# upb-lea/gym-electric-motor

Hardware: AMD Instinct MI355X
Metric: env-steps/sec (batched PMSM, tau=1e-4) (higher is better)
Workload: dtype f32; 1 GPU; Finite-CC-PMSM-v0 (Finite-B6C + dq transform), RK4, fp32, tau=1e-4, default constraint + auto-reset; 16384 envs/GPU x 1 GPU(s); one bench step = one fused launch of 1000 control steps, obs [K,N,S_out] rows + done bytes written for every control step; env_id=Finite-CC-PMSM-v0, envs_per_gpu=16384, solver=rk4, steps_per_launch=1000, parallelism=env-sharded x1, no data-path collective, world_size=1, oversubscribed=False

## Files before the change

### gym_electric_motor_amd/csrc/gemx_kernels.hpp

```cpp
#pragma once
#include <cstdio>

#include "gemx_common.hpp"

namespace gemx {

__device__ __forceinline__ float med3_r(float x, float lo, float hi) { return __builtin_amdgcn_fmed3f(x, lo, hi); }
__device__ __forceinline__ double med3_r(double x, double lo, double hi) { return fmin(fmax(x, lo), hi); }
template <class R> __device__ __forceinline__ R poly_load_ode(const DevParams<R> &P, R omega, R torque) {
    const R a = med3_r(P.lin_factor * omega, -P.la, P.la);
    const R tl = P.lc * (omega * fabs(omega)) + P.lb * omega + a;
    return (torque - tl) * P.inv_j;
}

template <int SYS, class R> struct Elec;

template <class R> struct Elec<GEMX_SYS_DC_PERMEX, R> {
    static constexpr int NM = 1;
    struct Pre { R b; };
    static __device__ __forceinline__ Pre prep(const DevParams<R> &P, R w, const R (&u)[MAX_U]) {
        const R bw = P.m[0] * w;
        return Pre{fma(P.m[2], u[0], bw)};
    }
    static __device__ __forceinline__ void f(const DevParams<R> &P, const Pre &p, const R (&x)[1], R (&dx)[1]) { dx[0] = p.b + P.m[1] * x[0]; }
// ... 485 lines not shown
                rhs(z, k1);
                wsum += rk_step_k1_pk<SOLVER, NP>(z, k1, hs, rhs);
            }
        }
        put();
        return P.pole * hs * wsum;
    }
    float deps = 0.0f;
    const float lim = P.omega_lim;
    const float h_td = hs * P.inv_tau_decay;
    for (int s = 0; s < (NS1 ? 1 : ns); ++s) {
        V k1;
        rhs(z, k1);
        const float w = z.w;
        const float wmid = fmaf(0.5f * hs, k1.w, w);
        const bool band = fabsf(wmid) < lim;
        const float c1 = band ? P.lin_factor : 0.0f, c0 = band ? 0.0f : copysignf(P.la, wmid);
        k1.w = fmaf(med3_r(P.lin_factor * w, -P.la, P.la) - fmaf(c1, w, c0), P.inv_j, k1.w);
        auto rhs_m = [&](const V &zz, V &dz) {
            const float om = zz.w;
            dz.w = (E.rhs(P, zz, dz) - (P.lc * (om * fabsf(om)) + P.lb * om + fmaf(c1, om, c0))) * P.inv_j;
        };
        float dw_end;
        deps += (P.pole * hs) * rk_step_k1_pk<SOLVER, NP>(z, k1, hs, rhs_m, &dw_end);
        const float w1 = z.w;
        const float phi_lim = copysignf(lim, wmid);
        const bool needs = (med3_r(w, -lim, lim) != (band ? w : phi_lim)) | (med3_r(w1, -lim, lim) != (band ? w1 : phi_lim));
        if (__any(needs)) {
            const float V0 = hs * k1.w, V1 = hs * dw_end, dl = w1 - w;
            const float c2 = 3.0f * dl - 2.0f * V0 - V1, c3 = V0 + V1 - 2.0f * dl;
            const KinkPath<float> kp{w, w1, V0, V0 * V0, 4.0f * (dl - V0), c2 * (1.0f / 3.0f), c3 * 0.25f, 0.5f * V0,
                                     w + 0.5f * V0 + c2 * (1.0f / 3.0f) + c3 * 0.25f, w1 > w};
            const float lev = (kp.up ? (w < -lim) : !(w > lim)) ? -lim : lim, oth = -lev;
            const float U1 = kp.ramp(lev);
            const bool o0 = w >= oth, o1 = w1 >= oth, full = o0 != o1;
            float U2 = (o0 & o1) ? kp.M - oth : 0.0f;
            if (__any(full)) {
                const float uf = kp.ramp(oth);
                U2 = full ? uf : U2;
            }
            const float Up = lev > 0.0f ? U1 : U2, Um = lev > 0.0f ? U2 : U1;
            const float D = -h_td * ((Um - Up - lim) - (band ? kp.M : phi_lim));
            z.w = w1 + (needs ? D : 0.0f);
        }
    }
    put();
    return deps;
}

template <int SYS>
__device__ __forceinline__ float dp5_adaptive_pk(const DevParams<float> &P, float (&y)[SysTraits<SYS>::ND], const float (&u)[MAX_U], float hs, float *hc) {
    constexpr int NP = pk_pairs<SYS>(), NZ = 1 + 2 * NP;
    using V = PkVec<NP>;
    const PkElec<SYS> E(P, u);
    V z, k1;
    z.w = y[0];
#pragma unroll
    for (int j = 0; j < NP; ++j) z.p[j] = f2_t{y[1 + 2 * j], y[2 + 2 * j]};
    auto rhs = [&](const V &zz, V &dz) { dz.w = poly_load_ode<float>(P, zz.w, E.rhs(P, zz, dz)); };
    const bool kink = P.kink_split != 0;
    V k1t;
    rhs(z, k1t);
    float t = 0.0f, h = dp5_first_try<float>(P, hs, hc), integral = 0.0f, hprop = 0.0f;
    const float hmin = hs * (1.0f / 1024.0f);
    bool gave_up = false;
#pragma nounroll
    for (int guard = 0; guard < 4096; ++guard) {
        const bool active = t < hs;
        if (!__any(active)) break;
        const bool fin = !(h < hs - t);
        const float hh = active ? (fin ? hs - t : h) : 0.0f;
        V k2, k3, k4, k5, k6, k7, zt, zn;
        k1 = k1t;
        float kc0 = 0.0f, kc1 = 0.0f, wmid = 0.0f;
        bool band = false;
        if (kink) {
            wmid = fmaf(0.5f * hh, k1t.w, z.w);
            band = fabsf(wmid) < P.omega_lim;
            kc1 = band ? P.lin_factor : 0.0f;
            kc0 = band ? 0.0f : copysignf(P.la, wmid);
            k1.w = fmaf(med3_r(P.lin_factor * z.w, -P.la, P.la) - fmaf(kc1, z.w, kc0), P.inv_j, k1t.w);
        }
        auto ev = [&](const V &zz, V &dz) {
            const float tq = E.rhs(P, zz, dz);
            const float om = zz.w;
            if (kink) dz.w = (tq - (P.lc * (om * fabsf(om)) + P.lb * om + fmaf(kc1, om, kc0))) * P.inv_j;
            else dz.w = poly_load_ode<float>(P, om, tq);
        };
        float q = (float)(35.0 / 384.0) * z.w;
        zt = pk_axpy(z, hh, pk_scale((float)(1.0 / 5.0), k1));
        ev(zt, k2);
        zt = pk_axpy(z, hh, pk_acc(pk_scale((float)(3.0 / 40.0), k1), (float)(9.0 / 40.0), k2));
        ev(zt, k3);
        q += (float)(500.0 / 1113.0) * zt.w;
        zt = pk_axpy(z, hh, pk_acc(pk_acc(pk_scale((float)(44.0 / 45.0), k1), -(float)(56.0 / 15.0), k2), (float)(32.0 / 9.0), k3));
        ev(zt, k4);
        q += (float)(125.0 / 192.0) * zt.w;
        zt = pk_axpy(z, hh, pk_acc(pk_acc(pk_acc(pk_scale((float)(19372.0 / 6561.0), k1), -(float)(25360.0 / 2187.0), k2), (float)(64448.0 / 6561.0), k3),
                                   -(float)(212.0 / 729.0), k4));
        ev(zt, k5);
        q -= (float)(2187.0 / 6784.0) * zt.w;
        zt = pk_axpy(z, hh, pk_acc(pk_acc(pk_acc(pk_acc(pk_scale((float)(9017.0 / 3168.0), k1), -(float)(355.0 / 33.0), k2), (float)(46732.0 / 5247.0), k3),
                                          (float)(49.0 / 176.0), k4), -(float)(5103.0 / 18656.0), k5));
        ev(zt, k6);
        q += (float)(11.0 / 84.0) * zt.w;
        zn = pk_axpy(z, hh, pk_acc(pk_acc(pk_acc(pk_acc(pk_scale((float)(35.0 / 384.0), k1), (float)(500.0 / 1113.0), k3), (float)(125.0 / 192.0), k4),
                                          -(float)(2187.0 / 6784.0), k5), (float)(11.0 / 84.0), k6));
        ev(zn, k7);
        const V er = pk_scale(hh, pk_acc(pk_acc(pk_acc(pk_acc(pk_acc(pk_scale((float)(71.0 / 57600.0), k1), -(float)(71.0 / 16695.0), k3), (float)(71.0 / 1920.0), k4),
                                                        -(float)(17253.0 / 339200.0), k5), (float)(22.0 / 525.0), k6), -(float)(1.0 / 40.0), k7));
        auto sq = [&](float e, float a0, float a1, float at) { const float r = e * rcp_r(at + P.rtol * fmaxf(fabsf(a0), fabsf(a1))); return r * r; };
        float e2 = sq(er.w, z.w, zn.w, P.atol_w);
#pragma unroll
        for (int j = 0; j < NP; ++j) e2 += sq(er.p[j].x, z.p[j].x, zn.p[j].x, P.atol) + sq(er.p[j].y, z.p[j].y, zn.p[j].y, P.atol);
        const float en2 = e2 * (1.0f / NZ);
        const bool floor_hit = !(hh > hmin);
        const bool accept = active && (!(en2 > 1.0f) || floor_hit);
        gave_up |= active && floor_hit && en2 > 1.0f;
        float fac = en2 > 1e-20f ? 0.9f * pow_m01(en2) : 10.0f;
        fac = fminf(fmaxf(fac, 0.2f), accept ? 10.0f : 1.0f);
        const float w0 = z.w;
        z.w = accept ? zn.w : z.w;
        k1t.w = accept ? k7.w : k1t.w;
#pragma unroll
        for (int j = 0; j < NP; ++j) {
            z.p[j] = accept ? zn.p[j] : z.p[j];
            k1t.p[j] = accept ? k7.p[j] : k1t.p[j];
        }
        if (kink) {
            const float lim = P.omega_lim, phi_lim = copysignf(lim, wmid), w1 = zn.w;
            const bool needs = accept && ((med3_r(w0, -lim, lim) != (band ? w0 : phi_lim)) | (med3_r(w1, -lim, lim) != (band ? w1 : phi_lim)));
            if (__any(needs)) {
                z.w = z.w + kink_defect<float>(P, w0, w1, hh * k1.w, hh * k7.w, wmid, band, needs, hh);
                V kt;
                rhs(z, kt);
                k1t.w = needs ? kt.w : k1t.w;
#pragma unroll
                for (int j = 0; j < NP; ++j) k1t.p[j] = needs ? kt.p[j] : k1t.p[j];
            }
        }
        integral += accept ? hh * q : 0.0f;
        t = accept ? (fin ? hs : t + hh) : t;
        h = active ? fmaxf(hh * fac, hmin) : h;
        hprop = accept ? fmaxf(hprop, h) : hprop;
    }
    if (gave_up && P.errw != nullptr) atomicOr(P.errw, (uint32_t)GEMX_ERRFLAG_TOLERANCE);
    if (dp5_carries<float>(P, hs, hc)) *hc = hprop;
    y[0] = z.w;
#pragma unroll
    for (int j = 0; j < NP; ++j) { y[1 + 2 * j] = z.p[j].x; y[2 + 2 * j] = z.p[j].y; }
    return integral;
}

template <int SYS, int LOAD, int SOLVER, class R, bool NS1 = false, bool LIN = false, int SEG = 0>
__device__ __forceinline__ R integrate(const DevParams<R> &P, R (&y)[SysTraits<SYS>::ND], const R (&u)[MAX_U], R h, const R *linr = nullptr, bool two = false,
                                       R *hc = nullptr) {
    using E = Elec<SYS, R>;
    constexpr int NM = E::NM;
    const int ns = NS1 ? 1 : P.nsteps;
    const R hs = NS1 ? h : h * P.inv_ns;
    if (LIN) {
        constexpr int NG = E::NG;
        R g[NG], x[NM];
        constexpr int NC = NM * (NM + NG);
        const R *L0 = linr != nullptr ? linr : P.lin + (SEG != 0 ? NC : 0);
        R L[NC];
        [[maybe_unused]] uint32_t two_mask = (SEG == 1 && two) ? 0xFFFFFFFFu : 0u;
        if constexpr (SEG == 1 && sizeof(R) == 4) asm volatile("" : "+v"(two_mask));
#pragma unroll
        for (int i = 0; i < NC; ++i) {
            if constexpr (SEG == 1 && sizeof(R) == 4) {
                uint32_t ca, cb;
                memcpy(&ca, &L0[2 * NC + i], 4);
                memcpy(&cb, &L0[i], 4);
                const uint32_t cs = (two_mask & cb) | (~two_mask & ca);
                memcpy(&L[i], &cs, 4);
            } else if constexpr (SEG == 1) {
                L[i] = two ? L0[i] : L0[2 * NC + i];
            } else {
                L[i] = L0[SEG == 2 ? NC + i : i];
            }
        }
        const R om = P.init[0];
        E::get_b(E::prep(P, om, u), g);
#pragma unroll
        for (int i = 0; i < NM; ++i) x[i] = y[1 + i];
        for (int s = 0; s < ns; ++s) {
            R xn[NM];
#pragma unroll
            for (int r = 0; r < NM; ++r) {
                constexpr bool X_FIRST = SEG == 0 && (SYS == GEMX_SYS_SYNC || SYS == GEMX_SYS_SCIM);
                constexpr bool X_LAST = !lin_phi_form<SYS, SEG>() && !X_FIRST;
                R acc = X_FIRST ? fma(L[NM * NM + r * NG], g[0], x[r]) : L[NM * NM + r * NG] * g[0];
#pragma unroll
                for (int i = 1; i < NG; ++i) acc += L[NM * NM + r * NG + i] * g[i];
#pragma unroll
                for (int c = 0; c < NM; ++c) acc += L[r * NM + c] * x[c];
                xn[r] = X_LAST ? x[r] + acc : acc;
            }
#pragma unroll
            for (int r = 0; r < NM; ++r) x[r] = xn[r];
        }
#pragma unroll
        for (int i = 0; i < NM; ++i) y[1 + i] = x[i];
        return P.pole * om * h;
    }
    if (LOAD == GEMX_LOAD_CONST_SPEED) {
        const typename E::Pre pre = E::prep(P, y[0], u);
        R x[NM];
#pragma unroll
        for (int i = 0; i < NM; ++i) x[i] = y[1 + i];
        auto rhs = [&](const R (&xx)[NM], R (&dx)[NM]) { E::f(P, pre, xx, dx); };
        if (SOLVER == GEMX_SOLVER_DP5 && P.adaptive) {
            dp5_adaptive<NM, R>(P, x, h, rhs, hc);
        } else if (NS1 || ns == 1) {
            rk_step<SOLVER, NM, R>(x, hs, rhs);
        } else {
            for (int s = 0; s < ns; ++s) rk_step<SOLVER, NM, R>(x, hs, rhs);
        }
#pragma unroll
        for (int i = 0; i < NM; ++i) y[1 + i] = x[i];
        return P.pole * y[0] * h;
    } else {
        if constexpr (sizeof(R) == 4 && pk_pairs<SYS>() > 0 && GEMX_PACKED_RHS) {
            if (!(SOLVER == GEMX_SOLVER_DP5 && P.adaptive)) return integrate_pk<SYS, SOLVER, NS1>(P, y, u, hs, ns);
            if constexpr (SOLVER == GEMX_SOLVER_DP5) return P.pole * dp5_adaptive_pk<SYS>(P, y, u, h, hc);
        }
        auto rhs = [&](const R (&z)[NM + 1], R (&dz)[NM + 1]) {
            R x[NM], dx[NM];
#pragma unroll
            for (int i = 0; i < NM; ++i) x[i] = z[1 + i];
            const typename E::Pre pre = E::prep(P, z[0], u);
            E::f(P, pre, x, dx);
            dz[0] = poly_load_ode(P, z[0], E::torque(P, x));
#pragma unroll
            for (int i = 0; i < NM; ++i) dz[1 + i] = dx[i];
        };
        if (SOLVER == GEMX_SOLVER_DP5 && P.adaptive) {
            auto rhs_mc = [&](const R (&z)[NM + 1], R (&dz)[NM + 1], R c0, R c1) {
                R x[NM], dx[NM];
#pragma unroll
                for (int i = 0; i < NM; ++i) x[i] = z[1 + i];
                const typename E::Pre pre = E::prep(P, z[0], u);
                E::f(P, pre, x, dx);
                dz[0] = (E::torque(P, x) - (P.lc * (z[0] * fabs(z[0])) + P.lb * z[0] + fma(c1, z[0], c0))) * P.inv_j;
#pragma unroll
                for (int i = 0; i < NM; ++i) dz[1 + i] = dx[i];
            };
            return P.pole * dp5_adaptive<NM + 1, R>(P, y, h, rhs, hc, rhs_mc);
        }
        if (!P.kink_split) {
            R wsum = R(0);
            if (NS1 || ns == 1) {
                wsum = rk_step<SOLVER, NM + 1, R>(y, hs, rhs);
            } else {
                for (int s = 0; s < ns; ++s) wsum += rk_step<SOLVER, NM + 1, R>(y, hs, rhs);
            }
            return P.pole * hs * wsum;
        }
        R deps = R(0);
        const R lim = P.omega_lim;
        const R h_td = hs * P.inv_tau_decay;
        for (int s = 0; s < ns; ++s) {
            R k1[NM + 1];
            rhs(y, k1);
            const R w = y[0];
            const R wmid = fma(R(0.5) * hs, k1[0], w);
            const bool band = fabs(wmid) < lim;
            const R c1 = band ? P.lin_factor : R(0), c0 = band ? R(0) : copysign(P.la, wmid);
            k1[0] = fma(med3_r(P.lin_factor * w, -P.la, P.la) - fma(c1, w, c0), P.inv_j, k1[0]);
            auto load_m = [&](R om, R torque) { return (torque - (P.lc * (om * fabs(om)) + P.lb * om + fma(c1, om, c0))) * P.inv_j; };
            auto rhs_m = [&](const R (&z)[NM + 1], R (&dz)[NM + 1]) {
                R x[NM], dx[NM];
#pragma unroll
                for (int i = 0; i < NM; ++i) x[i] = z[1 + i];
                const typename E::Pre pre = E::prep(P, z[0], u);
                E::f(P, pre, x, dx);
                dz[0] = load_m(z[0], E::torque(P, x));
#pragma unroll
                for (int i = 0; i < NM; ++i) dz[1 + i] = dx[i];
            };
            R dw_end;
            deps += (P.pole * hs) * rk_step_k1<SOLVER, NM + 1, R>(y, k1, hs, rhs_m, &dw_end);
            const R w1 = y[0];
            const R phi_lim = copysign(lim, wmid);
            const bool needs = (med3_r(w, -lim, lim) != (band ? w : phi_lim)) | (med3_r(w1, -lim, lim) != (band ? w1 : phi_lim));
#ifdef GEMX_KINK_NO_DEFECT
            if (false) {
#else
            if (__any(needs)) {
#endif
                const R V0 = hs * k1[0], V1 = hs * dw_end, dl = w1 - w;
                const R c2 = R(3) * dl - R(2) * V0 - V1, c3 = V0 + V1 - R(2) * dl;
                const KinkPath<R> kp{w, w1, V0, V0 * V0, R(4) * (dl - V0), c2 * R(1.0 / 3.0), c3 * R(0.25), R(0.5) * V0,
                                     w + R(0.5) * V0 + c2 * R(1.0 / 3.0) + c3 * R(0.25), w1 > w};
                const R lev = (kp.up ? (w < -lim) : !(w > lim)) ? -lim : lim, oth = -lev;
                const R U1 = kp.ramp(lev);
                const bool o0 = w >= oth, o1 = w1 >= oth, full = o0 != o1;
                R U2 = (o0 & o1) ? kp.M - oth : R(0);
                if (__any(full)) {
                    const R uf = kp.ramp(oth);
                    U2 = full ? uf : U2;
                }
                const R Up = lev > R(0) ? U1 : U2, Um = lev > R(0) ? U2 : U1;
                const R D = -h_td * ((Um - Up - lim) - (band ? kp.M : phi_lim));
                y[0] = w1 + (needs ? D : R(0));
            }
        }
        return deps;
    }
}

template <int SYS, class R, bool LIN>
__device__ __forceinline__ void elec_input(const DevParams<R> &P, R om, const R (&u)[MAX_U], const R *L, R (&in)[Elec<SYS, R>::NM]) {
    using E = Elec<SYS, R>;
    constexpr int NM = E::NM, NG = E::NG;
    static_assert(NG == NM, "the DC machines' affine part has one entry per state");
    R g[NG];
    E::get_b(E::prep(P, om, u), g);
#pragma unroll
    for (int r = 0; r < NM; ++r) {
        if (LIN) {
            R acc = L[NM * NM + r * NG] * g[0];
#pragma unroll
            for (int i = 1; i < NG; ++i) acc += L[NM * NM + r * NG + i] * g[i];
            in[r] = acc;
        } else {
            in[r] = g[r];
        }
    }
}
template <int SYS, int SOLVER, class R, bool LIN>
__device__ __forceinline__ void elec_apply(const DevParams<R> &P, R om, R (&x)[Elec<SYS, R>::NM], const R (&in)[Elec<SYS, R>::NM], const R *L) {
    using E = Elec<SYS, R>;
    constexpr int NM = E::NM;
    if (LIN) {
        R xn[NM];
#pragma unroll
        for (int r = 0; r < NM; ++r) {
            R acc = in[r];
#pragma unroll
            for (int c = 0; c < NM; ++c) acc += L[r * NM + c] * x[c];
            xn[r] = acc;
        }
#pragma unroll
        for (int r = 0; r < NM; ++r) x[r] = xn[r];
    } else {
        const R zu[MAX_U] = {R(0), R(0), R(0), R(0)};
        const typename E::Pre pre = E::set_b(E::prep(P, om, zu), in);
        auto rhs = [&](const R (&xx)[NM], R (&dx)[NM]) { E::f(P, pre, xx, dx); };
        rk_step<SOLVER, NM, R>(x, P.tau, rhs);
    }
}

template <bool IL, class R> __device__ __forceinline__ R cont_leg(const DevParams<R> &P, R duty, R i) {
// ... 67 lines not shown
    t32(c * ud - s * uq, s * ud + c * uq, act[0], act[1], act[2]);
    if (CONV == CONV_CONT_B6_4QC_DQ) act[3] = ue;
}

template <class R, bool LIN, int SEG>
__device__ __forceinline__ typename Angle<R>::T advance_angle(const DevParams<R> &P, typename Angle<R>::T ang, R deps, bool two) {
    if constexpr (LIN && SEG == 1) {
        const R w = P.pole * P.init[0];
        const typename Angle<R>::Inc i_il = Angle<R>::increment(w * P.t_il), i_tau = Angle<R>::increment(w * P.tau);
        return Angle<R>::add(ang, two ? i_il : i_tau);
    } else {
        return Angle<R>::advance(ang, deps);
    }
}

template <int SYS, int CONV, int LOAD, int SOLVER, bool IL, class R> struct Stepper;

template <int SYS, int CONV, int LOAD, int SOLVER, bool IL, class R> struct DcStepper {
    using AngT = typename Angle<R>::T;
    static constexpr int ND = SysTraits<SYS>::ND, NOUT = SysTraits<SYS>::NOUT, NC = ND - 1;
    static constexpr int NU = SYS == GEMX_SYS_DC_EXTEX ? 2 : 1;
    static constexpr int NH = NU;
    static constexpr int NVT = 0;
    static constexpr int row_slot(int j) { return j; }
    static constexpr bool CONT = CONV == GEMX_CONV_CONT_4QC || CONV == GEMX_CONV_CONT_2X4QC;
    static __device__ __forceinline__ uint32_t legs_of(uint32_t dact) {
        uint32_t legs = 0;
        if (!CONT) {
#pragma unroll
            for (int j = 0; j < NU; ++j) {
                const uint32_t aj = (dact >> (2 * j)) & 3u;
                legs |= (((aj & 2u) ? 2u : 1u) | (((aj & 1u) ? 2u : 1u) << 2)) << (4 * j);
            }
        }
        return legs;
    }
    static_assert((CONV == GEMX_CONV_CONT_2X4QC || CONV == GEMX_CONV_FINITE_2X4QC) == (NU == 2), "system / converter width mismatch");
    static __device__ __forceinline__ R i_in(const R (&y)[ND], int j) {
        if (SYS == GEMX_SYS_DC_EXTEX) return y[1 + j];
        return SYS == GEMX_SYS_DC_SHUNT ? y[1] + y[ND - 1] : y[1];
    }
    static __device__ __forceinline__ void input_voltages(const DevParams<R> &P, const R (&act)[MAX_ACT], uint32_t dact, R (&u)[MAX_U]) {
#pragma unroll
        for (int j = 0; j < NU; ++j) {
            if (CONT) {
                u[j] = (duty_pos(act[j]) - duty_neg(act[j])) * P.u_sup;
            } else {
                const uint32_t aj = (dact >> (2 * j)) & 3u;
                u[j] = (((aj & 2u) ? R(0) : R(1)) - ((aj & 1u) ? R(0) : R(1))) * P.u_sup;
            }
        }
    }
    template <bool NS1 = false, bool LIN = false, bool TAB = false>
    static __device__ __forceinline__ void advance(const DevParams<R> &P, R (&y)[ND], AngT &, uint32_t &sw, const R (&act)[MAX_ACT], uint32_t dact,
                                                   R (&ho)[NH], const R * = nullptr, const R *linr = nullptr, R *hc = nullptr) {
        R u[MAX_U] = {R(0), R(0), R(0), R(0)};
        if (CONT) {
#pragma unroll
            for (int j = 0; j < NU; ++j) {
                const R d0 = duty_pos(act[j]);
                const R d1 = duty_neg(act[j]);
                const R i = i_in(y, j);
                u[j] = (cont_leg<IL, R>(P, d0, i) - cont_leg<IL, R>(P, d1, i)) * P.u_sup;
            }
            integrate<SYS, LOAD, SOLVER, R, NS1, LIN, IL ? 1 : 0>(P, y, u, P.tau, linr, false, hc);
        } else {
            uint32_t legs = 0;
#pragma unroll
            for (int j = 0; j < NU; ++j) {
                const uint32_t aj = (dact >> (2 * j)) & 3u;
                legs |= (((aj & 2u) ? 2u : 1u) | (((aj & 1u) ? 2u : 1u) << 2)) << (4 * j);
            }
            bool two = false;
            if (IL) {
                if (P.t_il > R(0)) legs = b6_interlock<2 * NU>(sw, legs, two);
                sw = legs;
            }
            auto segment = [&](R h, auto seg_tag) {
#pragma unroll
                for (int j = 0; j < NU; ++j) {
                    const uint32_t s0 = (legs >> (4 * j)) & 3u, s1 = (legs >> (4 * j + 2)) & 3u;
                    R v0, v1;
                    if (!IL) {
                        v0 = s0 == 1u ? R(1) : R(0);
                        v1 = s1 == 1u ? R(1) : R(0);
                    } else {
                        const R i = i_in(y, j);
                        v0 = ((s0 == 1u) | ((s0 == 0u) & (i < R(0)))) ? R(1) : R(0);
                        v1 = ((s1 == 1u) | ((s1 == 0u) & (-i < R(0)))) ? R(1) : R(0);
                    }
                    u[j] = (v0 - v1) * P.u_sup;
                }
                integrate<SYS, LOAD, SOLVER, R, NS1, LIN, decltype(seg_tag)::value>(P, y, u, h, linr, two, hc);
            };
            if (IL) {
                segment(two ? P.t_il : P.tau, std::integral_constant<int, 1>{});
                if (two) segment(P.tau - P.t_il, std::integral_constant<int, 2>{});
            } else {
                segment(P.tau, std::integral_constant<int, 0>{});
            }
        }
#pragma unroll
        for (int j = 0; j < NU; ++j) ho[j] = u[j];
    }
    static __device__ __forceinline__ void observe(const DevParams<R> &P, const R (&y)[ND], AngT, const R (&ho)[NH], R (&obs)[NOUT]) {
        R x[NC];
#pragma unroll
        for (int c = 0; c < NC; ++c) x[c] = y[1 + c];
        obs[0] = y[0] * P.inv_lim[0];
        obs[1] = Elec<SYS, R>::torque(P, x) * P.inv_lim[1];
#pragma unroll
        for (int c = 0; c < NC; ++c) obs[2 + c] = y[1 + c] * P.inv_lim[2 + c];
#pragma unroll
        for (int j = 0; j < NU; ++j) obs[2 + NC + j] = ho[j] * P.inv_lim[2 + NC + j];
        obs[2 + NC + NU] = P.u_sup * P.inv_lim[2 + NC + NU];
    }
    static __device__ __forceinline__ bool default_done(const R (&obs)[NOUT]) {
        bool d = false;
#pragma unroll
        for (int c = 0; c < NC; ++c) d |= fabs(obs[2 + c]) > R(1);
        return d;
    }
    static __device__ __forceinline__ R state_violation(const DevParams<R> &P, const R (&y)[ND], const R (&)[NH]) {
        R v = fabs(y[1] * P.inv_lim[2]);
#pragma unroll
        for (int c = 1; c < NC; ++c) v = fmax(v, fabs(y[1 + c] * P.inv_lim[2 + c]));
        return v;
    }
};
template <int CONV, int LOAD, int SOLVER, bool IL, class R>
struct Stepper<GEMX_SYS_DC_PERMEX, CONV, LOAD, SOLVER, IL, R> : DcStepper<GEMX_SYS_DC_PERMEX, CONV, LOAD, SOLVER, IL, R> {};
template <int CONV, int LOAD, int SOLVER, bool IL, class R>
struct Stepper<GEMX_SYS_DC_SERIES, CONV, LOAD, SOLVER, IL, R> : DcStepper<GEMX_SYS_DC_SERIES, CONV, LOAD, SOLVER, IL, R> {};
template <int CONV, int LOAD, int SOLVER, bool IL, class R>
struct Stepper<GEMX_SYS_DC_SHUNT, CONV, LOAD, SOLVER, IL, R> : DcStepper<GEMX_SYS_DC_SHUNT, CONV, LOAD, SOLVER, IL, R> {};
template <int CONV, int LOAD, int SOLVER, bool IL, class R>
struct Stepper<GEMX_SYS_DC_EXTEX, CONV, LOAD, SOLVER, IL, R> : DcStepper<GEMX_SYS_DC_EXTEX, CONV, LOAD, SOLVER, IL, R> {};

template <int CONV, int LOAD, int SOLVER, bool IL, class R> struct Stepper<GEMX_SYS_SYNC, CONV, LOAD, SOLVER, IL, R> {
    using AngT = typename Angle<R>::T;
    static constexpr int NH = 7;
    static __device__ __forceinline__ uint32_t legs_of(uint32_t dact) { return CONV == GEMX_CONV_FINITE_B6 ? b6_subactions(dact) : 0u; }
    static constexpr int NVT = (CONV == GEMX_CONV_FINITE_B6 && !IL) ? 5 : 0;
    static constexpr int row_slot(int j) {
        constexpr int slot[12] = {2, 0, 1, 3, 4, 5, 8, 9, 10, 6, 7, 11};
        return j < 12 ? slot[j] : j;
    }
    static __device__ __forceinline__ void action_entry(const DevParams<R> &P, uint32_t dact, R (&e)[8]) {
        const R zero[MAX_ACT] = {R(0), R(0), R(0), R(0), R(0), R(0)};
        b6_voltages<CONV, false, R>(P, zero, dact, 0u, R(0), R(0), R(0), e[2], e[3], e[4]);
        t23(e[2], e[3], e[4], e[0], e[1]);
        e[5] = e[6] = e[7] = R(0);
    }
    template <bool NS1 = false, bool LIN = false, bool TAB = false>
    static __device__ __forceinline__ void advance(const DevParams<R> &P, R (&y)[3], AngT &ang, uint32_t &sw, const R (&act)[MAX_ACT],
                                                   uint32_t dact, R (&ho)[NH], const R *tab = nullptr, const R *linr = nullptr, R *hc = nullptr) {
        R s, c;
        Angle<R>::sincos(ang, s, c);
        uint32_t legs = 0;
        bool two = false;
        if (IL && CONV == GEMX_CONV_FINITE_B6) {
            legs = b6_subactions_packed(dact);
            if (P.t_il > R(0)) legs = b6_interlock(sw, legs, two);
            sw = legs;
        }
        R ua, ub, uc, u[MAX_U] = {R(0), R(0), R(0), R(0)};
        auto segment = [&](R h, auto seg_tag) {
            R ia = R(0), ib = R(0), ic = R(0);
            if (IL) {
                const R ial = c * y[1] - s * y[2], ibe = s * y[1] + c * y[2];
                t32(ial, ibe, ia, ib, ic);
            }
            R ual, ube;
            if (TAB) {
                ual = tab[0]; ube = tab[1]; ua = tab[2]; ub = tab[3]; uc = tab[4];
            } else {
                b6_voltages<CONV, IL, R>(P, act, dact, legs, ia, ib, ic, ua, ub, uc);
                t23(ua, ub, uc, ual, ube);
            }
            u[0] = c * ual + s * ube;
            u[1] = -s * ual + c * ube;
            const R deps = integrate<GEMX_SYS_SYNC, LOAD, SOLVER, R, NS1, LIN, decltype(seg_tag)::value>(P, y, u, h, linr, two, hc);
            ang = advance_angle<R, LIN, decltype(seg_tag)::value>(P, ang, deps, two);
        };
        if (IL) {
            segment(two ? P.t_il : P.tau, std::integral_constant<int, 1>{});
            if (two) {
                Angle<R>::sincos(ang, s, c);
                segment(P.tau - P.t_il, std::integral_constant<int, 2>{});
            }
        } else {
            segment(P.tau, std::integral_constant<int, 0>{});
        }
        ho[0] = s; ho[1] = c; ho[2] = ua; ho[3] = ub; ho[4] = uc; ho[5] = u[0]; ho[6] = u[1];
    }
    static __device__ __forceinline__ void observe(const DevParams<R> &P, const R (&y)[3], AngT ang, const R (&ho)[NH], R (&obs)[14]) {
        const R s = ho[0], c = ho[1];
        const R ial = c * y[1] - s * y[2], ibe = s * y[1] + c * y[2];
        R ia, ib, ic;
        t32(ial, ibe, ia, ib, ic);
        const R x[2] = {y[1], y[2]};
        obs[0] = y[0] * P.inv_lim[0];
        obs[1] = Elec<GEMX_SYS_SYNC, R>::torque(P, x) * P.inv_lim[1];
        obs[2] = ia * P.inv_lim[2];
        obs[3] = ib * P.inv_lim[3];
        obs[4] = ic * P.inv_lim[4];
        obs[5] = y[1] * P.inv_lim[5];
        obs[6] = y[2] * P.inv_lim[6];
        obs[7] = ho[2] * P.inv_lim[7];
        obs[8] = ho[3] * P.inv_lim[8];
        obs[9] = ho[4] * P.inv_lim[9];
        obs[10] = ho[5] * P.inv_lim[10];
        obs[11] = ho[6] * P.inv_lim[11];
        obs[12] = Angle<R>::wrapped(ang) * P.inv_lim[12];
        obs[13] = P.u_sup * P.inv_lim[13];
    }
    static __device__ __forceinline__ bool default_done(const R (&obs)[14]) { return obs[5] * obs[5] + obs[6] * obs[6] > R(1); }
    static __device__ __forceinline__ R state_violation(const DevParams<R> &P, const R (&y)[3], const R (&)[NH]) {
        const R o5 = y[1] * P.inv_lim[5], o6 = y[2] * P.inv_lim[6];
        return o5 * o5 + o6 * o6;
    }
};

template <int CONV, int LOAD, int SOLVER, bool IL, class R> struct Stepper<GEMX_SYS_EESM, CONV, LOAD, SOLVER, IL, R> {
    using AngT = typename Angle<R>::T;
    static constexpr int NH = 6;
    static __device__ __forceinline__ uint32_t legs_of(uint32_t) { return 0u; }
    static constexpr int B6 = CONV == GEMX_CONV_CONT_B6_4QC ? GEMX_CONV_CONT_B6 : GEMX_CONV_FINITE_B6;
    static __device__ __forceinline__ void voltages(const DevParams<R> &P, const R (&act)[MAX_ACT], uint32_t dact, R &ua, R &ub, R &uc, R &ue) {
        b6_voltages<B6, false, R>(P, act, dact & 7u, 0u, R(0), R(0), R(0), ua, ub, uc);
        if (CONV == GEMX_CONV_CONT_B6_4QC) {
            ue = (duty_pos(act[3]) - duty_neg(act[3])) * P.u_sup;
        } else {
            const uint32_t a1 = (dact >> 3) & 3u;
            ue = (((a1 & 2u) ? R(0) : R(1)) - ((a1 & 1u) ? R(0) : R(1))) * P.u_sup;
        }
    }
    static constexpr int NVT = CONV == GEMX_CONV_FINITE_B6_4QC ? 6 : 0;
    static constexpr int row_slot(int j) { return j; }
    static __device__ __forceinline__ void action_entry(const DevParams<R> &P, uint32_t dact, R (&e)[8]) {
        const R zero[MAX_ACT] = {R(0), R(0), R(0), R(0), R(0), R(0)};
        voltages(P, zero, dact, e[0], e[1], e[2], e[5]);
        t23(e[0], e[1], e[2], e[3], e[4]);
        e[6] = e[7] = R(0);
    }
    template <bool NS1 = false, bool LIN = false, bool TAB = false>
    static __device__ __forceinline__ void advance(const DevParams<R> &P, R (&y)[4], AngT &ang, uint32_t &, const R (&act)[MAX_ACT],
                                                   uint32_t dact, R (&ho)[NH], const R *tab = nullptr, const R *linr = nullptr, R *hc = nullptr) {
        R s, c;
        Angle<R>::sincos(ang, s, c);
        R ua, ub, uc, ue, u[MAX_U] = {R(0), R(0), R(0), R(0)};
        R ual, ube;
        if (TAB) {
            ua = tab[0]; ub = tab[1]; uc = tab[2]; ual = tab[3]; ube = tab[4]; ue = tab[5];
        } else {
            voltages(P, act, dact, ua, ub, uc, ue);
            t23(ua, ub, uc, ual, ube);
        }
        u[0] = c * ual + s * ube;
        u[1] = -s * ual + c * ube;
        u[2] = ue;
        const R deps = integrate<GEMX_SYS_EESM, LOAD, SOLVER, R, NS1, LIN, IL ? 1 : 0>(P, y, u, P.tau, linr, false, hc);
        ang = Angle<R>::advance(ang, deps);
        ho[0] = s; ho[1] = c; ho[2] = ua; ho[3] = ub; ho[4] = uc; ho[5] = ue;
    }
    static __device__ __forceinline__ void observe(const DevParams<R> &P, const R (&y)[4], AngT ang, const R (&ho)[NH], R (&obs)[16]) {
        const R s = ho[0], c = ho[1];
        const R ial = c * y[1] - s * y[2], ibe = s * y[1] + c * y[2];
        R ia, ib, ic;
        t32(ial, ibe, ia, ib, ic);
        const R x[3] = {y[1], y[2], y[3]};
        obs[0] = y[0] * P.inv_lim[0];
        obs[1] = Elec<GEMX_SYS_EESM, R>::torque(P, x) * P.inv_lim[1];
        obs[2] = ia * P.inv_lim[2];
        obs[3] = ib * P.inv_lim[3];
        obs[4] = ic * P.inv_lim[4];
        obs[5] = y[1] * P.inv_lim[5];
        obs[6] = y[2] * P.inv_lim[6];
        obs[7] = y[3] * P.inv_lim[7];
        obs[8] = ho[2] * P.inv_lim[8];
        obs[9] = ho[3] * P.inv_lim[9];
        obs[10] = ho[4] * P.inv_lim[10];
        R ual, ube;
        t23(ho[2], ho[3], ho[4], ual, ube);
        obs[11] = (c * ual + s * ube) * P.inv_lim[11];
        obs[12] = (-s * ual + c * ube) * P.inv_lim[12];
        obs[13] = ho[5] * P.inv_lim[13];
        obs[14] = Angle<R>::wrapped(ang) * P.inv_lim[14];
        obs[15] = P.u_sup * P.inv_lim[15];
    }
    static __device__ __forceinline__ bool default_done(const R (&obs)[16]) {
        return (obs[5] * obs[5] + obs[6] * obs[6] > R(1)) | (fabs(obs[7]) > R(1));
    }
    static __device__ __forceinline__ R state_violation(const DevParams<R> &P, const R (&y)[4], const R (&)[NH]) {
        const R o5 = y[1] * P.inv_lim[5], o6 = y[2] * P.inv_lim[6], o7 = y[3] * P.inv_lim[7];
        return fmax(o5 * o5 + o6 * o6, fabs(o7));
    }
};

template <int CONV, int LOAD, int SOLVER, bool IL, class R> struct Stepper<GEMX_SYS_SCIM, CONV, LOAD, SOLVER, IL, R> {
    using AngT = typename Angle<R>::T;
    static constexpr int NH = 5;
    static __device__ __forceinline__ uint32_t legs_of(uint32_t dact) { return CONV == GEMX_CONV_FINITE_B6 ? b6_subactions(dact) : 0u; }
    static constexpr int NVT = (CONV == GEMX_CONV_FINITE_B6 && !IL) ? 5 : 0;
    static constexpr int row_slot(int j) { return j; }
    static __device__ __forceinline__ void action_entry(const DevParams<R> &P, uint32_t dact, R (&e)[8]) {
        const R zero[MAX_ACT] = {R(0), R(0), R(0), R(0), R(0), R(0)};
        b6_voltages<CONV, false, R>(P, zero, dact, 0u, R(0), R(0), R(0), e[0], e[1], e[2]);
        t23(e[0], e[1], e[2], e[3], e[4]);
        e[5] = e[6] = e[7] = R(0);
    }
    static __device__ __forceinline__ void field_angle(R pa, R pb, R &s, R &c) { flux_angle<R>(pa, pb, s, c); }
    template <bool NS1 = false, bool LIN = false, bool TAB = false>
    static __device__ __forceinline__ void advance(const DevParams<R> &P, R (&y)[5], AngT &ang, uint32_t &sw, const R (&act)[MAX_ACT],
                                                   uint32_t dact, R (&ho)[NH], const R *tab = nullptr, const R *linr = nullptr, R *hc = nullptr) {
        R s, c;
        field_angle(y[3], y[4], s, c);
        uint32_t legs = 0;
        bool two = false;
        if (IL && CONV == GEMX_CONV_FINITE_B6) {
            legs = b6_subactions_packed(dact);
            if (P.t_il > R(0)) legs = b6_interlock(sw, legs, two);
            sw = legs;
        }
        R ua, ub, uc, u[MAX_U] = {R(0), R(0), R(0), R(0)};
        auto segment = [&](R h, auto seg_tag) {
            R ia = R(0), ib = R(0), ic = R(0);
            if (IL) t32(y[1], y[2], ia, ib, ic);
            if (TAB) {
                ua = tab[0]; ub = tab[1]; uc = tab[2]; u[0] = tab[3]; u[1] = tab[4];
            } else {
                b6_voltages<CONV, IL, R>(P, act, dact, legs, ia, ib, ic, ua, ub, uc);
                t23(ua, ub, uc, u[0], u[1]);
            }
// ... 1240 lines not shown
            }
            if (conv_dq<CONV>() && P.dq_processor) dq_action_stage<SYS, CONV, R>(P, y, ang, act);
            if constexpr (MODE == 3) {
                const bool one_deep = P.delay == 1, queued = since >= delay_u;
#pragma unroll
                for (int i = 0; i < NACTC; ++i) {
                    const R t = act[i];
                    qw[i] = t;
                    const R q = one_deep ? tprev[i] : qpre[i];
                    tprev[i] = t;
                    act[i] = queued ? q : P.dreset[i];
                    qpre[i] = qnext[i];
                }
            }
            if (FIFO && P.delay > 0) {
                R *f = fifo + ((size_t)slot * BLOCK + tid) * NACTC;
                slot = slot + 1 == P.delay ? 0 : slot + 1;
                const R *fn = fifo + ((size_t)slot * BLOCK + tid) * NACTC;
                const bool one_deep = P.delay == 1;
                if (DISCRETE) {
                    const R pushed = (R)dact;
                    f[0] = pushed;
                    dact = (uint32_t)pop[0];
                    pop[0] = one_deep ? pushed : fn[0];
                } else {
#pragma unroll
                    for (int i = 0; i < NACTC; ++i) {
                        const R pushed = act[i];
                        f[i] = pushed;
                        act[i] = pop[i];
                        pop[i] = one_deep ? pushed : fn[i];
                    }
                }
            }
            if (conv_dq<CONV>() && !P.dq_processor) dq_action_stage<SYS, CONV, R>(P, y, ang, act);
            R ho[NH];
            auto run_advance = [&](const DevParams<R> &Q) {
                if constexpr (TAB) {
                    ST::template advance<true, LINABLE, true>(Q, y, ang, sw, act, dact, ho, tab, linc, &hcar);
                } else {
                    if constexpr (FIFO && SLOW) {
                        if (!ns1) { ST::template advance<false, false>(Q, y, ang, sw, act, dact, ho, nullptr, nullptr, &hcar); return; }
                    }
                    if (LINABLE && (!FIFO || lin_ok)) ST::template advance<true, LINABLE>(Q, y, ang, sw, act, dact, ho, nullptr, linc);
                    else ST::template advance<true, false>(Q, y, ang, sw, act, dact, ho, nullptr, nullptr, &hcar);
                }
            };
            R gviol = R(0);
            auto generic_violation = [&](const DevParams<R> &Q) {
                if constexpr (FIFO && SLOW) {
                    if (generic_constr) {
                        R ob[NOUT];
                        ST::observe(Q, y, ang, ho, ob);
                        R lim = R(0), sq = R(0);
#pragma unroll
                        for (int i = 0; i < NOUT; ++i) {
                            lim = fmax(lim, P.cw[i] * fabs(ob[i]));
                            sq += (P.cw[GEMX_MAX_OUT + i] * ob[i]) * ob[i];
                        }
                        gviol = fmax(lim, sq);
                    }
                }
            };
            R usup_lane = P.u_sup;
            if constexpr (FULL) {
                DevParams<R> PL = P;
                if (P.rc_supply) {
                    const R isup = supply_current<SYS, conv_base<CONV>(), R>(P, y, ang, sw, act);
                    sup[0] = sup[0] + (P.u_sup - sup[0] - P.sup_r * isup) * P.sup_inv_rc * sup[1];
                    sup[1] = P.tau;
                    PL.u_sup = sup[0];
                }
                usup_lane = PL.u_sup;
                run_advance(PL);
                generic_violation(PL);
                if (!IL && conv_has_legs<CONV>() && P.rc_supply) sw = ST::legs_of(dact);
            } else {
                run_advance(P);
                generic_violation(P);
            }
            R viol = ST::state_violation(P, y, ho);
            if constexpr (FIFO && SLOW) viol = generic_constr ? gviol : viol;
            const bool done = viol > thr_done;
            constexpr bool COMPACT_ROW = COMPACT_K && TAB;
            if constexpr (COMPACT_ROW) {
                const uint32_t pk = (done ? 0x100u : 0u) | dact;
                R pkf, bits;
                memcpy(&pkf, &pk, sizeof(R));
                memcpy(&bits, &ang, sizeof(R));
                row[0] = y[1]; row[1] = y[2]; row[2] = pkf; row[3] = bits;
                row[4] = ho[0]; row[5] = ho[1]; row[6] = ho[5]; row[7] = ho[6];
            } else {
#pragma unroll
                for (int j = 0; j < ND; ++j) row[ST::row_slot(j)] = y[j];
                if (HAS_ANGLE) {
                    R bits;
                    memcpy(&bits, &ang, sizeof(R));
                    row[ST::row_slot(ND)] = bits;
                }
#pragma unroll
                for (int j = 0; j < NH; ++j) row[ST::row_slot(ND + (HAS_ANGLE ? 1 : 0) + j)] = ho[j];
                row[ST::row_slot(NDONE)] = done ? R(1) : R(0);
                if constexpr (FULL) row[ST::row_slot(NDONE + 1)] = usup_lane;
            }
            const bool rs = viol > thr_reset;
            constexpr bool OMEGA_FIXED = LINABLE && MODE != 1;
#pragma unroll
            for (int j = OMEGA_FIXED ? 1 : 0; j < ND; ++j) y[j] = rs ? init_v[j] : y[j];
            ang = rs ? init_ang_v : ang;
            if constexpr (SOLVER == GEMX_SOLVER_DP5) hcar = rs ? R(0) : hcar;
            if constexpr (FULL) {
#if defined(GEMX_AB_NO_RINIT_BLOCK)
                if constexpr (false) if (rs) {
#else
                if constexpr (RINIT) if (rs) {
#endif
#if defined(GEMX_AB_NO_INLINE)
                    if (true) {
#else
                    if (GEMX_PREP_DRAWS != 0 && GEMX_EXPECT_PREPARED(pre_hi.w == rcount + 1u)) {
#endif
                        const uint32_t w8[8] = {pre_lo.x, pre_lo.y, pre_lo.z, pre_lo.w, pre_hi.x, pre_hi.y, pre_hi.z, pre_hi.w};
#pragma unroll
                        for (int j = 0; j < ND; ++j) memcpy(&y[j], &w8[j], sizeof(R));
                        if (HAS_ANGLE) memcpy(&ang, &w8[ND], sizeof(R));
                        rcount += 1u;
#ifdef GEMX_TIMING
                        n_prepared += 1u;
#endif
                    } else {
                        draw_initial_state_cnt<SYS, R>(GEMX_PREP_DESC_COPY == 2 ? desc_lds : a.rinit, envc, rcount, y, ang);
#ifdef GEMX_TIMING
                        n_inline += 1u;
#endif
                    }
                    if (GEMX_PREP_DRAWS != 0) prep_cnt[tid] = rcount;
                    prefetch_draw();
                }
                sup[0] = rs ? P.u_sup : sup[0];
                sup[1] = rs ? R(0) : sup[1];
            }
            if constexpr (MODE == 2 || MODE == 3) since = rs ? 0u : (since < delay_u ? since + 1u : delay_u);
            if (FIFO && P.delay > 0) {
                if (rs) {
                    for (int d = 0; d < P.delay; ++d) {
#pragma unroll
                        for (int i = 0; i < NACTC; ++i) fifo[((size_t)d * BLOCK + tid) * NACTC + i] = P.dreset[i];
                    }
#pragma unroll
                    for (int i = 0; i < NACTC; ++i) pop[i] = P.dreset[i];
                }
            }
        };
        stage_actions(0);
        if (n_ref > 0) stage_refs(0);
        if (LW != 0 && DISCRETE) {
            __builtin_amdgcn_s_waitcnt(0x0F70);
            __syncthreads();
        }
#ifdef GEMX_TIMING
        unsigned long long tv = 0, tc = 0, tw = 0, tlong = 0, T0 = clock64(), W0 = wall_clock64(), t0, t0b, t1, t2;
#endif
        constexpr bool PIPE_PACED = !(D == PIPE_D && OW == PIPE_OUT_WAVES_RW);
        uint32_t pace = 0u;
        unsigned long long pace_t0 = 0ull;
        if constexpr (PIPE_PACED) {
            pace = blockIdx.x >= a.pace_tail_from ? a.pace_tail_ticks : a.pace_block_ticks;
            pace_t0 = pace != 0u ? wall_clock64() : 0ull;
        }
        for (int b = 0; b < nb; ++b) {
            if constexpr (PIPE_PACED) {
                if (pace != 0u) {
                    const unsigned long long due = pace_t0 + (unsigned long long)b * pace;
                    while (wall_clock64() < due) __builtin_amdgcn_s_sleep(4);
                }
            }
#ifdef GEMX_TIMING
            t0 = clock64();
#endif
            if constexpr (FULL) {
                if constexpr (RINIT) prefetch_draw();
            }
            const int sb = steps_of(b);
            R *hb = hand + (size_t)(b & 1) * D * BLOCK * NHT + (size_t)tid * NHT;
            __builtin_amdgcn_s_waitcnt(0x0F70);
#ifdef GEMX_TIMING
            t0b = clock64();
#endif
            if (LW == 0 && b + 1 < nb) {
                stage_actions(b + 1);
                if (n_ref > 0) stage_refs(b + 1);
            }
            R an[NACT], ac[NACT] = {};
            uint32_t dn = 0, dc = 0;
#pragma unroll
            for (int i = 0; i < NACT; ++i) an[i] = R(0);
            auto read_delayed = [&](int s, R (&dst)[NACT], uint32_t &ddst) {
                if (s >= P.delay) {
                    read_action(b, s - P.delay, dst, ddst);
                } else {
                    const R *c = fifo + ((size_t)s * BLOCK + tid) * NACTC;
                    if (DISCRETE) ddst = (uint32_t)c[0];
                    else {
#pragma unroll
                        for (int i = 0; i < NACT; ++i) dst[i] = c[i];
                    }
                }
            };
            [[maybe_unused]] constexpr uint32_t AMASK = DISCRETE ? (uint32_t)(ConvTraits<CONV>::NACTIONS - 1) : 0u;
            [[maybe_unused]] auto fetch_entry = [&](uint32_t d, R (&e)[8]) {
                const R *src = vtab + (size_t)(d & AMASK) * 8;
#pragma unroll
                for (int j = 0; j < 8; ++j) e[j] = j < ST::NVT ? src[j] : R(0);
            };
            auto run_block = [&](auto delayed_tag, auto ns_tag) {
                constexpr bool DEL = decltype(delayed_tag)::value;
                constexpr int NS = decltype(ns_tag)::value;
                using Mode = std::integral_constant<int, DEL ? 2 : 0>;
                auto rd = [&](int s, R (&dst)[NACT], uint32_t &ddst) {
                    if constexpr (DEL) read_delayed(s, dst, ddst);
                    else read_action(b, s, dst, ddst);
                };
                rd(0, an, dn);
                if constexpr (USE_TAB) {
                    R en[8], ec[8], e0[8];
                    uint32_t dnn = 0;
                    if constexpr (DEL) fetch_entry(P.dreset_d, e0);
                    fetch_entry(dn, en);
                    rd(1, an, dnn);
#pragma unroll 4
                    for (int s = 0; s < NS; ++s) {
                        dc = dn;
#pragma unroll
                        for (int j = 0; j < 8; ++j) ec[j] = en[j];
                        dn = dnn;
                        fetch_entry(dn, en);
                        rd(s + 2 < NS ? s + 2 : NS - 1, an, dnn);
                        if constexpr (DEL) {
                            const bool queued = since >= delay_u;
#pragma unroll
                            for (int j = 0; j < ST::NVT; ++j) ec[j] = queued ? ec[j] : e0[j];
                            if constexpr (COMPACT_K) dc = queued ? dc : P.dreset_d;
                        }
                        one_step(Mode{}, ac, dc, hb + (size_t)s * BLOCK * NHT, ec);
                    }
                } else {
#pragma unroll 4
                    for (int s = 0; s < NS; ++s) {
                        dc = dn;
#pragma unroll
                        for (int i = 0; i < NACT; ++i) ac[i] = an[i];
                        rd(s + 1 < NS ? s + 1 : s, an, dn);
                        if constexpr (DEL) {
                            const bool queued = since >= delay_u;
                            dc = queued ? dc : P.dreset_d;
#pragma unroll
                            for (int i = 0; i < NACT; ++i) ac[i] = queued ? ac[i] : (i < NACTC ? P.dreset[i < NACTC ? i : 0] : R(0));
                        }
                        one_step(Mode{}, ac, dc, hb + (size_t)s * BLOCK * NHT, nullptr);
                    }
                }
            };
            bool compact_blk = false;
            using WholeBlock = std::integral_constant<int, D>;
            constexpr bool TAIL48 = D == PIPE_D && PIPE_D == 12 && SYS == GEMX_SYS_SYNC;
            if ((sb == D || (TAIL48 && (sb == 4 || sb == 8))) && P.delay == 0 && (!LINABLE || lin_ok) && !slow_path) {
                if (sb == D) run_block(std::false_type{}, WholeBlock{});
                else if constexpr (TAIL48) {
                    if (sb == 8) run_block(std::false_type{}, std::integral_constant<int, 8>{});
                    else run_block(std::false_type{}, std::integral_constant<int, 4>{});
                }
                compact_blk = COMPACT_K;
            } else if (CAN_DELAY && delayed) {
                compact_blk = COMPACT_K;
                if constexpr (CAN_DELAY) {
                    if (sb == D) {
                        run_block(std::true_type{}, WholeBlock{});
                    } else {
                        R ect[8] = {};
#pragma nounroll
                        for (int s = 0; s < sb; ++s) {
                            read_delayed(s, ac, dc);
                            const bool queued = since >= delay_u;
                            dc = queued ? dc : P.dreset_d;
#pragma unroll
                            for (int i = 0; i < NACT; ++i) ac[i] = queued ? ac[i] : (i < NACTC ? P.dreset[i < NACTC ? i : 0] : R(0));
                            if constexpr (USE_TAB) fetch_entry(dc, ect);
                            one_step(std::integral_constant<int, 2>{}, ac, dc, hb + (size_t)s * BLOCK * NHT, ect);
                        }
                    }
                    for (int j = 0; j < P.delay; ++j) {
                        const int idx = j + sb - P.delay;
                        R *c = fifo + ((size_t)j * BLOCK + tid) * NACTC;
                        R v[NACTC];
#pragma unroll
                        for (int i = 0; i < NACTC; ++i) v[i] = R(0);
                        if (idx >= 0) {
                            R t[NACT];
                            uint32_t td = 0;
#pragma unroll
                            for (int i = 0; i < NACT; ++i) t[i] = R(0);
                            read_action(b, idx, t, td);
                            if (DISCRETE) v[0] = (R)(td & AMASK);
                            else {
#pragma unroll
                                for (int i = 0; i < NACT; ++i) v[i] = t[i];
                            }
                        } else {
                            const R *o = fifo + ((size_t)(j + sb) * BLOCK + tid) * NACTC;
#pragma unroll
                            for (int i = 0; i < NACTC; ++i) v[i] = o[i];
                        }
#pragma unroll
                        for (int i = 0; i < NACTC; ++i) c[i] = v[i];
                    }
                }
            } else if (CAN_DELAY && delayed_t) {
                if constexpr (CAN_DELAY && conv_dq<CONV>()) {
                    auto qrow = [&](int r) { return fifo + ((size_t)r * BLOCK + tid) * NACTC; };
                    using Mode3 = std::integral_constant<int, 3>;
                    read_action(b, 0, an, dn);
                    if (sb == D) {
#pragma unroll 4
                        for (int s = 0; s < D; ++s) {
#pragma unroll
                            for (int i = 0; i < NACT; ++i) ac[i] = an[i];
                            read_action(b, s + 1 < D ? s + 1 : s, an, dn);
                            one_step(Mode3{}, ac, 0u, hb + (size_t)s * BLOCK * NHT, nullptr, qrow(s + P.delay), qrow(s + 1));
                        }
                    } else {
#pragma nounroll
                        for (int s = 0; s < sb; ++s) {
#pragma unroll
                            for (int i = 0; i < NACT; ++i) ac[i] = an[i];
                            read_action(b, s + 1 < sb ? s + 1 : s, an, dn);
                            one_step(Mode3{}, ac, 0u, hb + (size_t)s * BLOCK * NHT, nullptr, qrow(s + P.delay), qrow(s + 1));
                        }
                    }
                    for (int j = 0; j < P.delay; ++j) {
                        R v[NACTC];
#pragma unroll
                        for (int i = 0; i < NACTC; ++i) v[i] = qrow(sb + j)[i];
#pragma unroll
                        for (int i = 0; i < NACTC; ++i) qrow(j)[i] = v[i];
                    }
                }
            } else {
                read_action(b, 0, an, dn);
#pragma nounroll
                for (int s = 0; s < sb; ++s) {
                    dc = dn;
#pragma unroll
                    for (int i = 0; i < NACT; ++i) ac[i] = an[i];
                    read_action(b, s + 1 < sb ? s + 1 : s, an, dn);
                    one_step(std::integral_constant<int, 1>{}, ac, dc, hb + (size_t)s * BLOCK * NHT, nullptr);
                }
            }
            if constexpr (COMPACT_K) {
                if (tid == 0) vtab[6 + (b & 1)] = compact_blk ? R(1) : R(0);
            }
#ifdef GEMX_TIMING
            t1 = clock64();
#endif
            __syncthreads();
#ifdef GEMX_TIMING
            t2 = clock64();
            tv += t0b - t0; tc += t1 - t0b; tw += t2 - t1;
            tlong += (t2 - t1) > 1000 ? 1 : 0;
            if (blockIdx.x == 0 && tid == 0 && b >= 100 && b < 148) {
                unsigned long long *tr = reinterpret_cast<unsigned long long *>(reinterpret_cast<char *>(a.err) + 64) + 64 + 0 * 96 + 2 * (b - 100);
                tr[0] = t1; tr[1] = t2;
            }
#endif
        }
#ifdef GEMX_TIMING
// ... 1251 lines not shown
```

Measured before the change: 113.6 billion env-steps/s.

## Add speculative pipelined fast path for compact float linear PMSM steps

Adds a specialized per-step path for the compact float case. It precomputes the next step's sincos, inverse Park voltages and linear-map inputs for both the continue and reset branches, then selects between them branch-free after the constraint check. Action reads and voltage-table lookups are prefetched several steps ahead, and each row is written with the packed done/action bits. The aim is to shorten the serial dependency chain per control step, at the cost of duplicate work on the reset branch, more registers and a separate code path that has to match the generic semantics.

After: 101.1 billion env-steps/s. -11.0%, worse.

```diff
diff --git a/gym_electric_motor_amd/csrc/gemx_kernels.hpp b/gym_electric_motor_amd/csrc/gemx_kernels.hpp
--- a/gym_electric_motor_amd/csrc/gemx_kernels.hpp
+++ b/gym_electric_motor_amd/csrc/gemx_kernels.hpp
@@ -661,6 +661,26 @@
     return integral;
 }
 
+template <int SYS, int SEG, class R>
+__device__ __forceinline__ void lin_map_apply(const R (&L)[Elec<SYS, R>::NM * (Elec<SYS, R>::NM + Elec<SYS, R>::NG)], const R (&g)[Elec<SYS, R>::NG],
+                                              R (&x)[Elec<SYS, R>::NM]) {
+    constexpr int NM = Elec<SYS, R>::NM, NG = Elec<SYS, R>::NG;
+    R xn[NM];
+#pragma unroll
+    for (int r = 0; r < NM; ++r) {
+        constexpr bool X_FIRST = SEG == 0 && (SYS == GEMX_SYS_SYNC || SYS == GEMX_SYS_SCIM);
+        constexpr bool X_LAST = !lin_phi_form<SYS, SEG>() && !X_FIRST;
+        R acc = X_FIRST ? fma(L[NM * NM + r * NG], g[0], x[r]) : L[NM * NM + r * NG] * g[0];
+#pragma unroll
+        for (int i = 1; i < NG; ++i) acc += L[NM * NM + r * NG + i] * g[i];
+#pragma unroll
+        for (int c = 0; c < NM; ++c) acc += L[r * NM + c] * x[c];
+        xn[r] = X_LAST ? x[r] + acc : acc;
+    }
+#pragma unroll
+    for (int r = 0; r < NM; ++r) x[r] = xn[r];
+}
+
 template <int SYS, int LOAD, int SOLVER, class R, bool NS1 = false, bool LIN = false, int SEG = 0>
 __device__ __forceinline__ R integrate(const DevParams<R> &P, R (&y)[SysTraits<SYS>::ND], const R (&u)[MAX_U], R h, const R *linr = nullptr, bool two = false,
                                        R *hc = nullptr) {
@@ -694,22 +714,7 @@
         E::get_b(E::prep(P, om, u), g);
 #pragma unroll
         for (int i = 0; i < NM; ++i) x[i] = y[1 + i];
-        for (int s = 0; s < ns; ++s) {
-            R xn[NM];
-#pragma unroll
-            for (int r = 0; r < NM; ++r) {
-                constexpr bool X_FIRST = SEG == 0 && (SYS == GEMX_SYS_SYNC || SYS == GEMX_SYS_SCIM);
-                constexpr bool X_LAST = !lin_phi_form<SYS, SEG>() && !X_FIRST;
-                R acc = X_FIRST ? fma(L[NM * NM + r * NG], g[0], x[r]) : L[NM * NM + r * NG] * g[0];
-#pragma unroll
-                for (int i = 1; i < NG; ++i) acc += L[NM * NM + r * NG + i] * g[i];
-#pragma unroll
-                for (int c = 0; c < NM; ++c) acc += L[r * NM + c] * x[c];
-                xn[r] = X_LAST ? x[r] + acc : acc;
-            }
-#pragma unroll
-            for (int r = 0; r < NM; ++r) x[r] = xn[r];
-        }
+        for (int s = 0; s < ns; ++s) lin_map_apply<SYS, SEG, R>(L, g, x);
 #pragma unroll
         for (int i = 0; i < NM; ++i) y[1 + i] = x[i];
         return P.pole * om * h;
@@ -1083,6 +1088,16 @@
         t23(e[2], e[3], e[4], e[0], e[1]);
         e[5] = e[6] = e[7] = R(0);
     }
+    static __device__ __forceinline__ void park_inv(R s, R c, R ual, R ube, R &ud, R &uq) {
+        ud = c * ual + s * ube;
+        uq = -s * ual + c * ube;
+    }
+    static __device__ __forceinline__ void lin_inputs(const DevParams<R> &P, R s, R c, R ual, R ube, R (&udq)[2], R (&g)[2]) {
+        R u[MAX_U] = {R(0), R(0), R(0), R(0)};
+        park_inv(s, c, ual, ube, u[0], u[1]);
+        Elec<GEMX_SYS_SYNC, R>::get_b(Elec<GEMX_SYS_SYNC, R>::prep(P, P.init[0], u), g);
+        udq[0] = u[0]; udq[1] = u[1];
+    }
     template <bool NS1 = false, bool LIN = false, bool TAB = false>
     static __device__ __forceinline__ void advance(const DevParams<R> &P, R (&y)[3], AngT &ang, uint32_t &sw, const R (&act)[MAX_ACT],
                                                    uint32_t dact, R (&ho)[NH], const R *tab = nullptr, const R *linr = nullptr, R *hc = nullptr) {
@@ -1109,8 +1124,7 @@
                 b6_voltages<CONV, IL, R>(P, act, dact, legs, ia, ib, ic, ua, ub, uc);
                 t23(ua, ub, uc, ual, ube);
             }
-            u[0] = c * ual + s * ube;
-            u[1] = -s * ual + c * ube;
+            park_inv(s, c, ual, ube, u[0], u[1]);
             const R deps = integrate<GEMX_SYS_SYNC, LOAD, SOLVER, R, NS1, LIN, decltype(seg_tag)::value>(P, y, u, h, linr, two, hc);
             ang = advance_angle<R, LIN, decltype(seg_tag)::value>(P, ang, deps, two);
         };
@@ -2657,6 +2671,49 @@
                 }
             }
         };
+        constexpr bool SPEC = COMPACT_K && std::is_same<R, float>::value;
+        [[maybe_unused]] R sp_s = R(0), sp_c = R(0), sp_sr = R(0), sp_cr = R(0);
+        [[maybe_unused]] typename Angle<R>::Inc sp_inc = typename Angle<R>::Inc(0);
+        if constexpr (SPEC) {
+            Angle<R>::sincos(ang, sp_s, sp_c);
+            Angle<R>::sincos(init_ang_v, sp_sr, sp_cr);
+            sp_inc = Angle<R>::increment(P.pole * P.init[0] * P.tau);
+        }
+        [[maybe_unused]] auto spec_step = [&](uint32_t dact, const R (&en)[2], R (&u)[2], R (&g)[2], R *row) {
+            if constexpr (SPEC) {
+                if (LW == 0) bad_action |= dact >= (uint32_t)ConvTraits<CONV>::NACTIONS;
+                dact &= (uint32_t)(ConvTraits<CONV>::NACTIONS - 1);
+                const AngT ang_c = Angle<R>::add(ang, sp_inc);
+                R s_c, c_c, u_c[2], g_c[2], u_r[2], g_r[2];
+                Angle<R>::sincos(ang_c, s_c, c_c);
+                ST::lin_inputs(P, s_c, c_c, en[0], en[1], u_c, g_c);
+                ST::lin_inputs(P, sp_sr, sp_cr, en[0], en[1], u_r, g_r);
+                R x[2] = {y[1], y[2]};
+                lin_map_apply<SYS, 0, R>(linc, g, x);
+                y[1] = x[0]; y[2] = x[1];
+                const R ho0[NH] = {};
+                R viol = ST::state_violation(P, y, ho0);
+                asm volatile("" : "+v"(viol), "+v"(s_c), "+v"(c_c), "+v"(u_c[0]), "+v"(u_c[1]), "+v"(g_c[0]), "+v"(g_c[1]), "+v"(u_r[0]), "+v"(u_r[1]),
+                             "+v"(g_r[0]), "+v"(g_r[1]));
+                const bool done = viol > thr_done;
+                const uint32_t pk = (done ? 0x100u : 0u) | dact;
+                R pkf, bits;
+                memcpy(&pkf, &pk, sizeof(R));
+                memcpy(&bits, &ang_c, sizeof(R));
+                row[0] = y[1]; row[1] = y[2]; row[2] = pkf; row[3] = bits;
+                row[4] = sp_s; row[5] = sp_c; row[6] = u[0]; row[7] = u[1];
+                const bool rs = viol > thr_reset;
+                const R x0 = x[0], x1 = x[1], i1 = init_v[1], i2 = init_v[2], sr = sp_sr, cr = sp_cr;
+                const R uc0 = u_c[0], uc1 = u_c[1], gc0 = g_c[0], gc1 = g_c[1], ur0 = u_r[0], ur1 = u_r[1], gr0 = g_r[0], gr1 = g_r[1];
+                const AngT ia = init_ang_v;
+                const R nx0 = rs ? i1 : x0, nx1 = rs ? i2 : x1, ns = rs ? sr : s_c, nc = rs ? cr : c_c;
+                const R nu0 = rs ? ur0 : uc0, nu1 = rs ? ur1 : uc1, ng0 = rs ? gr0 : gc0, ng1 = rs ? gr1 : gc1;
+                const AngT na = rs ? ia : ang_c;
+                y[1] = nx0; y[2] = nx1; ang = na; sp_s = ns; sp_c = nc;
+                u[0] = nu0; u[1] = nu1; g[0] = ng0; g[1] = ng1;
+                if constexpr (SOLVER == GEMX_SOLVER_DP5) hcar = rs ? R(0) : hcar;
+            }
+        };
         stage_actions(0);
         if (n_ref > 0) stage_refs(0);
         if (LW != 0 && DISCRETE) {
@@ -2726,6 +2783,31 @@
                     if constexpr (DEL) read_delayed(s, dst, ddst);
                     else read_action(b, s, dst, ddst);
                 };
+                if constexpr (SPEC) if constexpr (!DEL) {
+                    auto rda = [&](int s) {
+                        uint32_t d = 0;
+                        read_action(b, s < NS ? s : NS - 1, an, d);
+                        return d;
+                    };
+                    auto entry2 = [&](uint32_t d, R (&e)[2]) {
+                        const R *src = vtab + (size_t)(d & AMASK) * 8;
+                        e[0] = src[0]; e[1] = src[1];
+                    };
+                    uint32_t d0 = rda(0), d1 = rda(1), d2 = rda(2);
+                    R e0[2], e1[2], e2[2], u[2], g[2];
+                    entry2(d0, e0);
+                    entry2(d1, e1);
+                    ST::lin_inputs(P, sp_s, sp_c, e0[0], e0[1], u, g);
+#pragma unroll 4
+                    for (int s = 0; s < NS; ++s) {
+                        entry2(d2, e2);
+                        const uint32_t d3 = rda(s + 3);
+                        spec_step(d0, e1, u, g, hb + (size_t)s * BLOCK * NHT);
+                        d0 = d1; d1 = d2; d2 = d3;
+                        e1[0] = e2[0]; e1[1] = e2[1];
+                    }
+                    return;
+                }
                 rd(0, an, dn);
                 if constexpr (USE_TAB) {
                     R en[8], ec[8], e0[8];
```
